# abelxiaoxing/ImageClassification

Hardware: AMD Instinct MI355X
Metric: images/sec (whole node) ResNet-50 bf16 224^2 training (higher is better)
Workload: dtype bf16; 1 GPU; resnet50 train step, synthetic 3x224x224, batch 256/GPU, AdamW, label smoothing 0.1, 1000 classes (BASELINE configs[1]); global_batch=256, parallelism=dp1

## Files before the change

imageclassification_amd/csrc/capi.hip:

```cpp
#include "../../include/icamd.h"
#include "common.h"
#include "icamd_internal.h"
#include <cstdlib>
#include <string.h>

int icamd_bn_finalize_launch(const float* part, int nrows, int C, double count, const float* gamma, const float* beta,
                             float* running_mean, float* running_var, float momentum, float eps, float* mean,
                             float* invstd, float* scale, float* shift, double* chunks, hipStream_t s);
int icamd_bn_eval_coeffs_launch(int C, const float* gamma, const float* beta, const float* rm, const float* rv, float eps,
                                float* scale, float* shift, hipStream_t s);
int icamd_bn_apply_launch(const bf16_t* y, const float* scale, const float* shift, const bf16_t* residual, bf16_t* out,
                          unsigned char* maskbits, long long numel, int C, int relu, hipStream_t s,
                          const float* res_scale = nullptr, const float* res_shift = nullptr);
int icamd_bn_bwd_rows_per_block(long long rows, int C);
int icamd_bn_bwd_launch(const bf16_t* dout, const bf16_t* act, const bf16_t* y, const float* mean, const float* invstd,
                        const float* scale, const float* shift, float* dgamma, float* dbeta, bf16_t* dy, bf16_t* gout,
                        const unsigned char* maskbits, long long rows, int C, int relu, int accumulate, float* part,
                        double* chunks, float* c1c2, hipStream_t s, const unsigned char* pool_idx = nullptr,
                        int pool_ih = 0, int pool_iw = 0);
int icamd_bn_bwd_dual_launch(const bf16_t* dout, const unsigned char* maskbits, const bf16_t* yA, const float* meanA,
                             const float* invstdA, const float* scaleA, float* dgammaA, float* dbetaA, bf16_t* dyA,
                             const bf16_t* yB, const float* meanB, const float* invstdB, const float* scaleB, float* dgammaB,
                             float* dbetaB, bf16_t* dyB, long long rows, int C, int accumulate, float* partA, double* chunksA,
                             float* cA, float* partB, double* chunksB, float* cB, hipStream_t s);
// ... 404 lines not shown
  if (!conv_desc_ok(d) || d->KH != 1 || d->KW != 1 || d->stride != 1 || d->pad != 0) return 0;
  return icamd_pw_resident_bnred_wanted((long long)d->N * d->IH * d->IW, d->Cin, d->Cout) ? 1 : 0;
}

int icamd_conv2d_dgrad_bnred(const icamd_conv_desc* d, const void* dy, const void* w_t, void* g, const void* addend,
                             const uint8_t* addend_bits, int addend_sub2, const void* bn_y, const uint8_t* bn_bits,
                             float* partials, void* stream) {
  ProfScope _prof(PC_IGEMM_DGRAD, stream);
  const ConvWork cw = conv_work(d); _prof.work(cw.out + 3 * cw.in + 2 * cw.w + cw.in / 16 + (addend_bits ? cw.in / 16 : 0), cw.flops);
  if (!conv_desc_ok(d) || dy == nullptr || w_t == nullptr || g == nullptr || addend == nullptr || bn_y == nullptr ||
      bn_bits == nullptr || partials == nullptr || (addend_sub2 && addend_bits != nullptr))
    return ICAMD_ERR_BAD_ARG;
  if (!icamd_conv2d_dgrad_bnred_supported(d)) return ICAMD_ERR_UNSUPPORTED;
  PwResidentParams p;
  memset(&p, 0, sizeof(p));
  p.A = (const bf16_t*)dy; p.B = (const bf16_t*)w_t; p.out = (bf16_t*)g; p.addend = (const bf16_t*)addend;
  p.addend_bits = addend_bits;
  p.bn_y = (const bf16_t*)bn_y; p.bn_bits = bn_bits; p.bn_part = partials;
  p.M = d->N * d->IH * d->IW; p.N = d->Cin; p.K = d->Cout;
  if (addend_sub2) { p.sub2_h = d->IH; p.sub2_w = d->IW; }
  return icamd_pw_resident_bnred_launch(p, (hipStream_t)stream);
}

size_t icamd_conv2d_wgrad_workspace_bytes(const icamd_conv_desc* d) {
  if (!conv_desc_ok(d)) return 0;
  int S = 1, rows = 0;
  const long long M = (long long)d->N * d->OH * d->OW;
  if (M >= (1ll << 30)) return 0;
  const int Ktot = d->KH * d->KW * d->Cin;
  icamd_wgrad_plan((int)M, d->Cout, Ktot, &S, &rows);
  if (icamd_wgrad_halo_wanted(d->KH, d->KW, d->stride, d->pad, d->OH, d->OW, d->Cin, d->Cout, M)) {
    int S2 = 1;
    icamd_wgrad_halo_plan((int)M, d->Cin, d->Cout, &S2, &rows);
    if (S2 > S) S = S2;
  }
  return (size_t)S * d->Cout * ((size_t)Ktot + 1) * sizeof(float);
}

static int wgrad_impl(const icamd_conv_desc* d, const void* x, const void* dy, float* dw, float* dbias, int accumulate,
                      void* workspace, size_t workspace_bytes, void* stream);

int icamd_conv2d_wgrad(const icamd_conv_desc* d, const void* x, const void* dy, float* dw, int accumulate,
                       void* workspace, size_t workspace_bytes, void* stream) {
  ProfScope _prof(PC_WGRAD, stream);
  const ConvWork cw = conv_work(d); _prof.work(cw.in + cw.out + 4 * cw.w, cw.flops);
  return wgrad_impl(d, x, dy, dw, nullptr, accumulate, workspace, workspace_bytes, stream);
// ... 861 lines not shown
```

imageclassification_amd/csrc/conv3x3_halo.hip:

```cpp
#ifndef ICAMD_C64_NT
#define ICAMD_C64_NT 0
#endif
#include "common.h"
#include "icamd_internal.h"
#include <cstdlib>

namespace {

template <int N> __device__ __forceinline__ void halo_wait_vmcnt() {
  static_assert(N >= 0 && N < 64, "vmcnt is a 6-bit field");
  asm volatile("s_waitcnt vmcnt(%0)" ::"n"(N) : "memory");
}

__device__ __forceinline__ int swzq(int blk) { return (0x78 >> (2 * blk)) & 3; }

template <int BN, int WN, int MFR, int LA, int NB, int KS, int WPS>
__global__ __launch_bounds__(256, WPS) void conv3x3_halo_kernel(const Halo3x3Params p) {
  constexpr int WM = 4 / WN;
  constexpr int BM = WM * MFR * 16;
  constexpr int NJ = BN / WN / 16;
  constexpr int A_SLOTS = 4 * LA * 8;
  constexpr int ZERO_SLOT = A_SLOTS - 1;
  constexpr int A_BYTES = A_SLOTS * 128;
  constexpr int B_STAGE = BN * KS * 2;
  constexpr int LB = BN * KS / 2048;
  static_assert(KS == 32 || KS == 64, "filter stage width");
  constexpr int RING = NB * B_STAGE;
  constexpr int EPI_BYTES = BM * BN * 2;
  constexpr int LDS_BYTES = (A_BYTES + RING > EPI_BYTES) ? A_BYTES + RING : EPI_BYTES;
  static_assert(NB >= 2 && NB <= 8 && (WN == 1 || WN == 2) && LB >= 1, "configuration");
  __shared__ __attribute__((aligned(16))) unsigned char smem[LDS_BYTES];
  unsigned char* const sA = smem;
  unsigned char* const sB = smem + A_BYTES;

  const int tid = threadIdx.x, lane = tid & 63;
  const int wave = __builtin_amdgcn_readfirstlane(tid >> 6);
  const int wm = wave % WM, wn = wave / WM;
  const int fr = lane & 15, fq = lane >> 4;

// ... 151 lines not shown
  constexpr int ROWB = BN * 2, CPR = BN / 8;
#pragma unroll
  for (int j = 0; j < NJ; ++j) {
    const int cl = wn * (BN / WN) + j * 16 + 4 * fq;
    const int cg = n0 + cl;
    const int cgc = cg < p.Cout ? cg : 0;
    f32x4 b4 = {0.f, 0.f, 0.f, 0.f};
    if (p.bias != nullptr) b4 = *(const f32x4*)(p.bias + cgc);
#pragma unroll
    for (int i = 0; i < MFR; ++i) {
      const int ml = wm * (BM / WM) + i * 16 + fr;
      f32x4 v = acc[j][i] + b4;
      if (p.relu) {
#pragma unroll
        for (int e = 0; e < 4; ++e) v[e] = v[e] < 0.f ? 0.f : v[e];
      }
      u32x2 pk;
      pk[0] = pack_bf16x2(v[0], v[1]);
      pk[1] = pack_bf16x2(v[2], v[3]);
      const int slot = cl >> 2;
      *(u32x2*)(smem + ml * ROWB + ((((slot >> 1) ^ ml) & (CPR - 1)) << 4) + ((slot & 1) << 3)) = pk;
    }
  }
  __syncthreads();
  constexpr int RPP = 256 / CPR;
  constexpr int NPASS = BM / RPP;
  const int cp = tid & (CPR - 1), rg = tid / CPR;
  const int co = n0 + cp * 8;
  const bool co_ok = co < p.Cout;
  float s1[8], s2[8];
#pragma unroll
  for (int e = 0; e < 8; ++e) { s1[e] = 0.f; s2[e] = 0.f; }
#pragma unroll
  for (int ps = 0; ps < NPASS; ++ps) {
    const int ml = ps * RPP + rg;
    const int m = m0 + ml;
    const u32x4 o = *(const u32x4*)(smem + ml * ROWB + (((cp ^ ml) & (CPR - 1)) << 4));
    if (m < p.M && co_ok) {
      *(u32x4*)(p.out + (long long)m * p.Cout + co) = o;
      if (p.stats != nullptr) {
#pragma unroll
        for (int e = 0; e < 4; ++e) {
          const float lo = bf16_lo(o[e]), hi = bf16_hi(o[e]);
          s1[2 * e] += lo; s2[2 * e] += lo * lo;
          s1[2 * e + 1] += hi; s2[2 * e + 1] += hi * hi;
        }
      }
    }
  }
  if (p.stats != nullptr) {
    __syncthreads();
    float* red = (float*)smem;
#pragma unroll
    for (int e = 0; e < 8; ++e) {
      red[(rg * 2 + 0) * BN + cp * 8 + e] = s1[e];
      red[(rg * 2 + 1) * BN + cp * 8 + e] = s2[e];
    }
    __syncthreads();
    const int ntm = (p.M + BM - 1) / BM, nrows = (p.M + 127) / 128;
    for (int idx = tid; idx < 2 * BN; idx += 256) {
      const int which = idx / BN, c = idx - which * BN;
      float s = 0.f;
#pragma unroll 4
      for (int g = 0; g < RPP; ++g) s += red[(g * 2 + which) * BN + c];
      if (n0 + c < p.Cout) {
        p.stats[((long long)tile_m * 2 + which) * p.Cout + n0 + c] = s;
        if (ntm + tile_m < nrows) p.stats[((long long)(ntm + tile_m) * 2 + which) * p.Cout + n0 + c] = 0.f;
      }
    }
  }
}

template <bool ACT>
__global__ __launch_bounds__(256, 2) void conv3x3_c64_resident_kernel(const Halo3x3Params p, const int ntiles) {
  constexpr int BM = 128, LA = 8;
  constexpr int A_BYTES = 32 * LA * 128;
  constexpr int E_BYTES = 4 * 64 * 64;
  constexpr int ZERO_SLOT = 32 * LA - 1;
  __shared__ __attribute__((aligned(16))) unsigned char smem[2 * A_BYTES + E_BYTES];

  const int tid = threadIdx.x, lane = tid & 63;
  const int wave = __builtin_amdgcn_readfirstlane(tid >> 6);
  const int wm = wave & 1, wn = wave >> 1;
  const int fr = lane & 15, fq = lane >> 4;
  const int W = p.W, H = p.H;
  const bf16_t* __restrict__ in = p.in;
  const bf16_t* zero = (const bf16_t*)icamd_zero_page;
  unsigned char* const sE = smem + 2 * A_BYTES + wave * 4096;
  const unsigned lds_base = (unsigned)(uintptr_t)LPTR(smem);

  const int a_slot = wave * 8 + (lane >> 3);
  const int a_lc = (((lane & 7) - (lane >> 3)) & 7) * 8;
  const bool a_zero_lane = a_slot == 31;
  auto stage_a = [&](int m0, unsigned char* dst) {
    const int pix0 = m0 - (W + 1) + a_slot;
    const bf16_t* src0 = in + ((long long)pix0 * 64 + a_lc);
// ... 112 lines not shown
    for (int j = 0; j < 2; ++j) {
      f32x4 b4 = {0.f, 0.f, 0.f, 0.f};
      if constexpr (ACT) {
        if (p.bias != nullptr) b4 = *(const f32x4*)(p.bias + wn * 32 + j * 16 + 4 * fq);
      }
#pragma unroll
      for (int i = 0; i < 4; ++i) {
        const int pl = i * 16 + fr;
        f32x4 v = acc[j][i];
        if constexpr (ACT) {
          v += b4;
          if (p.relu) {
#pragma unroll
            for (int e = 0; e < 4; ++e) v[e] = v[e] < 0.f ? 0.f : v[e];
          }
        }
        u32x2 pk;
        pk[0] = pack_bf16x2(v[0], v[1]);
        pk[1] = pack_bf16x2(v[2], v[3]);
        const int slot = j * 4 + fq;
        *(u32x2*)(sE + pl * 64 + ((((slot >> 1) ^ (pl >> 2)) & 3) << 4) + ((slot & 1) << 3)) = pk;
      }
    }
    {
      const int pl0 = lane >> 2;
      const int mrow = m0 + wm * 64 + pl0;
      bf16_t* orow = p.out + ((long long)mrow * 64 + wn * 32 + (lane & 3) * 8);
      const bool want_stats = p.stats != nullptr;
#pragma unroll
      for (int r = 0; r < 4; ++r) {
        const int pl = r * 16 + pl0;
        const u32x4 o = *(const u32x4*)(sE + pl * 64 + ((((lane & 3) ^ (pl >> 2)) & 3) << 4));
        if (mrow + r * 16 < p.M) {
          *(u32x4*)(orow + r * (16 * 64)) = o;
          if (want_stats) {
#pragma unroll
            for (int e = 0; e < 4; ++e) {
              const f32x2 v = {bf16_lo(o[e]), bf16_hi(o[e])};
              s1[e] += v;
              s2[e] = __builtin_elementwise_fma(v, v, s2[e]);
            }
          }
        }
      }
    }
  }

  if (p.stats != nullptr) {
    __syncthreads();
    float* red = (float*)smem;
    const int g = wm * 16 + (lane >> 2);
    const int c0 = wn * 32 + (lane & 3) * 8;
#pragma unroll
    for (int e = 0; e < 4; ++e) {
      red[(g * 2 + 0) * 64 + c0 + 2 * e] = s1[e][0];
      red[(g * 2 + 0) * 64 + c0 + 2 * e + 1] = s1[e][1];
      red[(g * 2 + 1) * 64 + c0 + 2 * e] = s2[e][0];
      red[(g * 2 + 1) * 64 + c0 + 2 * e + 1] = s2[e][1];
    }
    __syncthreads();
    if (tid < 128) {
      const int which = tid >> 6, c = tid & 63;
      float s = 0.f;
#pragma unroll 8
      for (int k = 0; k < 32; ++k) s += red[(k * 2 + which) * 64 + c];
      p.stats[((long long)blockIdx.x * 2 + which) * 64 + c] = s;
      const int nrows = (p.M + 127) / 128;
      for (int r = blockIdx.x + gridDim.x; r < nrows; r += gridDim.x) p.stats[((long long)r * 2 + which) * 64 + c] = 0.f;
    }
  }
}

int launch_resident_c64(const Halo3x3Params& p, hipStream_t stream) {
  const int ntiles = (p.M + 127) / 128;
  const int slots = 2 * icamd_num_cus();
  const int grid = ntiles < slots ? ntiles : slots;
  if (p.bias != nullptr || p.relu)
    hipLaunchKernelGGL((conv3x3_c64_resident_kernel<true>), dim3((unsigned)grid), dim3(256), 0, stream, p, ntiles);
  else
    hipLaunchKernelGGL((conv3x3_c64_resident_kernel<false>), dim3((unsigned)grid), dim3(256), 0, stream, p, ntiles);
  return icamd_launch_status();
}

template <int BN, int WN, int MFR, int LA, int NB, int KS, int WPS>
int launch_halo(const Halo3x3Params& p, hipStream_t stream) {
  constexpr int BM = (4 / WN) * MFR * 16;
  const int ntm = (p.M + BM - 1) / BM;
  hipLaunchKernelGGL((conv3x3_halo_kernel<BN, WN, MFR, LA, NB, KS, WPS>), dim3((unsigned)(ntm * p.ntiles_n)), dim3(256), 0,
                     stream, p);
  return icamd_launch_status();
}

int halo_mode() {
  static const int m = [] { const char* e = getenv("ICAMD_CONV3X3_HALO"); return e ? atoi(e) : 1; }();
  return m;
}

}

static bool resident_c64_ok(int W, int C, int Cout) {
  static const int on = [] { const char* e = getenv("ICAMD_CONV3X3_RESIDENT"); return e ? atoi(e) : 1; }();
  return on != 0 && C == 64 && Cout == 64 && W % 8 == 0 && 128 + 2 * W + 2 <= 255;
}

bool icamd_halo3x3_wanted(int N, int H, int W, int C, int Cout) {
  if (halo_mode() == 0) return false;
  if (C % 64 != 0 || Cout % 8 != 0 || W < 3 || H < 3) return false;
  if (resident_c64_ok(W, C, Cout)) return true;
  if (halo_mode() == 1 && C < 256) return false;
  if ((long long)N * H * W >= (1ll << 30)) return false;
  if (2 * W + 3 + 128 > 4 * 8 * 8) return false;
  return true;
}

int icamd_halo3x3_launch(Halo3x3Params& p, hipStream_t stream) {
  if (!icamd_halo3x3_wanted(p.N, p.H, p.W, p.C, p.Cout)) return ICAMD_ERR_UNSUPPORTED;
  p.M = p.N * p.H * p.W;
  p.divHW = make_fastdiv((unsigned)(p.H * p.W));
  p.divW = make_fastdiv((unsigned)p.W);
  if (resident_c64_ok(p.W, p.C, p.Cout)) return launch_resident_c64(p, stream);
  const int bn = p.Cout <= 64 ? 64 : 128;
  p.ntiles_n = (p.Cout + bn - 1) / bn;
  int bm = 128;
  if (halo_mode() == 3) bm = 256;
  else if (halo_mode() != 2) {
    long long best = -1;
    for (int cand : {256, 224, 128}) {
      if (cand == 224 && bn != 128) continue;
      if ((cand + 2 * p.W + 3 + 31) / 32 > (cand == 128 ? 8 : 12)) continue;
      const long long tiles = (long long)((p.M + cand - 1) / cand) * p.ntiles_n;
      const long long cost = ((tiles + 511) / 512) * cand + (cand == 128 ? 16 : 0);
      if (best < 0 || cost < best) { best = cost; bm = cand; }
    }
  }
  const bool big = bm != 128;
  const int slots = bm + 2 * p.W + 2 + 1;
  const int la = (slots + 31) / 32;
  if (la > 12) return ICAMD_ERR_UNSUPPORTED;
  if (bn == 128) {
// ... 24 lines not shown
```

imageclassification_amd/csrc/icamd_internal.h:

```cpp
#pragma once
#include "common.h"

#define ICAMD_MAX_TAPS 56

struct IgemmParams {
  const bf16_t* in;
  const bf16_t* wt;
  bf16_t* out;
  const bf16_t* addend;
  const unsigned char* addend_bits;
  int addend_sub2;
  const float* bias;
  float* stats;
  const bf16_t* bnb_y;
  const bf16_t* bnb_mask;
  const float *bnb_mean, *bnb_invstd, *bnb_scale, *bnb_shift;
  int bnb_relu;
  int relu;
  bf16_t* gelu_out;
  int gelu_inplace;
  const bf16_t* gelu_z;
  int N, IH, IW, Cin;
  int OH, OW, Cout;
  int P, Q, M;
  int ostr, ooff_h, ooff_w, istr;
  int ntaps, Ktot;
  int KW, pad;
  int tap_sign, regular_taps;
  int stem7;
  int ksteps, ntiles_n;
  FastDiv divPQ, divQ, divCin, divKW;
  short dh[ICAMD_MAX_TAPS], dw[ICAMD_MAX_TAPS], wtap[ICAMD_MAX_TAPS];
};
int icamd_igemm_launch(IgemmParams& p, hipStream_t stream);
int icamd_igemm_pick_bn(int Cout);

struct Halo3x3Params {
  const bf16_t* in;
  const bf16_t* wt;
  bf16_t* out;
  const float* bias;
  float* stats;
  int relu;
  int flip;
  int N, H, W, C, Cout;
  int M, ntiles_n;
  FastDiv divHW, divW;
};
bool icamd_halo3x3_wanted(int N, int H, int W, int C, int Cout);
int icamd_halo3x3_launch(Halo3x3Params& p, hipStream_t stream);

struct GConvParams {
  const bf16_t* in;
  const bf16_t* w;
  bf16_t* out;
  const bf16_t* dy;
  float* slab;
  const float* bias;
  float* stats;
  int relu;
  int N, IH, IW, OH, OW, C, groups, stride;
  int Cg, M, npix_in, nalloc;
  int S, tiles_per_split, ntiles;
  FastDiv divOHW, divOW;
};
bool icamd_gconv3x3_ok(int N, int IH, int IW, int OH, int OW, int C, int groups, int stride);
int icamd_gconv3x3_fwd_launch(GConvParams& p, hipStream_t stream);
int icamd_gconv3x3_dgrad_launch(GConvParams& p, hipStream_t stream);
size_t icamd_gconv3x3_wgrad_bytes(int N, int IH, int IW, int OH, int OW, int C, int groups, int stride);
int icamd_gconv3x3_wgrad_launch(GConvParams& p, hipStream_t stream);

struct GemmNtParams {
// ... 128 lines not shown
```

imageclassification_amd/hip.py:

```python
import ctypes
import os
from ctypes import POINTER, Structure, c_double, c_float, c_int, c_longlong, c_size_t, c_void_p

import torch

_HERE = os.path.dirname(os.path.abspath(__file__))
LIB_PATH = os.path.join(_HERE, "csrc", "libicamd.so")

ABI_VERSION = 6
ERRORS = {1: "ICAMD_ERR_BAD_ARG", 2: "ICAMD_ERR_UNSUPPORTED", 3: "ICAMD_ERR_WORKSPACE", 4: "ICAMD_ERR_LAUNCH"}


class IcamdError(RuntimeError):
    pass


class BnBwdFuse(Structure):
    _fields_ = [("y", c_void_p), ("mask_src", c_void_p), ("mean", c_void_p), ("invstd", c_void_p), ("scale", c_void_p),
                ("shift", c_void_p), ("partials", c_void_p), ("relu", c_int)]


class ImageDesc(Structure):
    _fields_ = [("src_offset", ctypes.c_int64), ("src_h", c_int), ("src_w", c_int), ("crop_top", c_int), ("crop_left", c_int),
                ("crop_h", c_int), ("crop_w", c_int), ("hflip", c_int), ("vflip", c_int), ("jitter_order", c_int * 3),
# ... 19 lines not shown


def conv_desc(N, IH, IW, Cin, Cout, KH, KW, stride, pad):
    OH = (IH + 2 * pad - KH) // stride + 1
    OW = (IW + 2 * pad - KW) // stride + 1
    return ConvDesc(N, IH, IW, Cin, OH, OW, Cout, KH, KW, stride, pad)


_P = c_void_p
_SIGNATURES = {
    "icamd_abi_version": (c_int, []),
    "icamd_conv2d_fwd_gelu": (c_int, [_P, _P, _P, _P, _P, _P, _P]),
    "icamd_conv2d_dgrad_gelu": (c_int, [_P, _P, _P, _P, _P, _P]),
    "icamd_conv2d_fwd_act": (c_int, [_P, _P, _P, _P, _P, _P, c_int, _P]),
    "icamd_bn_fold_filters": (c_int, [_P, _P, _P, _P, _P, c_float, c_int, c_int, _P, _P, _P]),
    "icamd_conv2d_stats_rows": (c_int, [POINTER(ConvDesc)]),
    "icamd_conv2d_fwd": (c_int, [POINTER(ConvDesc), _P, _P, _P, _P, _P, _P, _P]),
    "icamd_conv2d_dgrad": (c_int, [POINTER(ConvDesc), _P, _P, _P, _P, _P, _P]),
    "icamd_conv2d_dgrad_sub2": (c_int, [POINTER(ConvDesc), _P, _P, _P, _P, _P]),
    "icamd_conv2d_dgrad_stats_rows": (c_int, [POINTER(ConvDesc)]),
    "icamd_conv2d_dgrad_bnbwd": (c_int, [POINTER(ConvDesc), _P, _P, _P, _P, POINTER(BnBwdFuse), _P]),
    "icamd_conv2d_dgrad_bnred_supported": (c_int, [POINTER(ConvDesc)]),
    "icamd_conv2d_dgrad_bnred": (c_int, [POINTER(ConvDesc), _P, _P, _P, _P, _P, c_int, _P, _P, _P, _P]),
    "icamd_bn_bwd_from_gy_partials": (c_int, [_P, c_int, _P, _P, _P, _P, _P, _P, _P, _P, c_longlong, c_int, c_int, _P, c_size_t, _P]),
    "icamd_bn_apply_conv1x1_fused_supported": (c_int, [POINTER(ConvDesc)]),
    "icamd_bn_apply_conv1x1_fused": (c_int, [POINTER(ConvDesc), _P, _P, _P, _P, _P, _P, _P, _P, _P, _P, _P, _P]),
    "icamd_conv1x1_bn_bwd_fused_supported": (c_int, [POINTER(ConvDesc)]),
    "icamd_conv1x1_bn_bwd_fused_workspace_bytes": (c_size_t, [POINTER(ConvDesc)]),
    "icamd_conv1x1_bn_bwd_fused": (c_int, [POINTER(ConvDesc), _P, c_int, _P, _P, _P, _P, _P, _P, _P, _P, _P, _P, _P, c_int, _P, c_size_t,
                                           _P, c_size_t, _P]),
    "icamd_conv2d_wgrad_workspace_bytes": (c_size_t, [POINTER(ConvDesc)]),
    "icamd_conv2d_wgrad": (c_int, [POINTER(ConvDesc), _P, _P, _P, c_int, _P, c_size_t, _P]),
    "icamd_conv2d_wgrad_bias": (c_int, [POINTER(ConvDesc), _P, _P, _P, _P, c_int, _P, c_size_t, _P]),
    "icamd_gconv3x3_supported": (c_int, [POINTER(ConvDesc), c_int]),
    "icamd_gconv3x3_fwd": (c_int, [POINTER(ConvDesc), c_int, _P, _P, _P, _P, _P]),
    "icamd_gconv3x3_fwd_act": (c_int, [POINTER(ConvDesc), c_int, _P, _P, _P, _P, c_int, _P]),
    "icamd_gconv3x3_dgrad": (c_int, [POINTER(ConvDesc), c_int, _P, _P, _P, _P]),
    "icamd_gconv3x3_wgrad_workspace_bytes": (c_size_t, [POINTER(ConvDesc), c_int]),
    "icamd_gconv3x3_wgrad": (c_int, [POINTER(ConvDesc), c_int, _P, _P, _P, c_int, _P, c_size_t, _P]),
    "icamd_filter_transpose": (c_int, [_P, _P, _P, _P, c_int, _P]),
    "icamd_filter_transpose_tiled": (c_int, [_P, _P, _P, _P, c_int, _P]),
    "icamd_bn_workspace_bytes": (c_size_t, [c_int]),
    "icamd_bn_train_finalize": (c_int, [_P, c_int, c_int, c_double, _P, _P, _P, _P, c_float, c_float, _P, _P, _P, _P, _P, _P]),
    "icamd_bn_eval_coeffs": (c_int, [c_int, _P, _P, _P, _P, c_float, _P, _P, _P]),
    "icamd_bn_apply": (c_int, [_P, _P, _P, _P, _P, _P, c_longlong, c_int, c_int, _P]),
    "icamd_bn_apply_res_bn": (c_int, [_P, _P, _P, _P, _P, _P, _P, _P, c_longlong, c_int, c_int, _P]),
# ... 135 lines not shown
```

imageclassification_amd/nets.py:

```python
import ctypes
import math
import os
from collections import OrderedDict

import torch

from . import hip
from .checkpoint import PicklableModel

BN_EPS = 1e-5
_FUSED_BNBWD = os.environ.get("ICAMD_FUSED_BNBWD", "0") == "1"
_WGRAD_STREAM = os.environ.get("ICAMD_WGRAD_STREAM", "1") != "0"
_DUAL_BNBWD = os.environ.get("ICAMD_DUAL_BNBWD", "1") != "0"
_SUB2_SHORTCUT = os.environ.get("ICAMD_SUB2_SHORTCUT", "1") != "0"
_FUSED_POOL_BWD = os.environ.get("ICAMD_FUSED_POOL_BWD", "1") != "0"
BN_MOMENTUM = 0.1

ARCHS = {
    "resnet18": ("basic", [2, 2, 2, 2], 1, 64),
    "resnet34": ("basic", [3, 4, 6, 3], 1, 64),
    "resnet50": ("bottleneck", [3, 4, 6, 3], 1, 64),
    "resnet101": ("bottleneck", [3, 4, 23, 3], 1, 64),
    "resnet152": ("bottleneck", [3, 8, 36, 3], 1, 64),
    "wide_resnet50_2": ("bottleneck", [3, 4, 6, 3], 1, 128),
    "wide_resnet101_2": ("bottleneck", [3, 4, 23, 3], 1, 128),
    "resnext50_32x4d": ("bottleneck", [3, 4, 6, 3], 32, 4),
    "resnext101_32x4d": ("bottleneck", [3, 4, 23, 3], 32, 4),
}


def block_specs(arch):
    block, layers, cardinality, base_width = ARCHS[arch]
    expansion = 4 if block == "bottleneck" else 1
    specs = []
    inplanes = 64
    for li, (planes, nblocks) in enumerate(zip([64, 128, 256, 512], layers)):
        for bi in range(nblocks):
            stride = 2 if (bi == 0 and li > 0) else 1
# ... 417 lines not shown
        ws = self._ws.get(key)
        if ws is not None:
            return ws
        dev = self.device
        lib = self.lib
        ws = {"N": N, "H": H, "W": W}

        def act(n, h, w, c):
            return torch.empty(n, h, w, c, dtype=torch.bfloat16, device=dev)

        Ws = W + (W & 1)
        ws["Ws"] = Ws
        ws["x8"] = act(N, H, Ws + 8, 4)
        d0 = self.stem_conv.desc(N, H, Ws)
        ws["y0"] = act(N, d0.OH, d0.OW, 64)
        ws["a0"] = act(N, d0.OH, d0.OW, 64)
        PH, PW = (d0.OH - 1) // 2 + 1, (d0.OW - 1) // 2 + 1
        ws["p0"] = act(N, PH, PW, 64)
        ws["p0_idx"] = torch.empty(N, PH, PW, 64, dtype=torch.uint8, device=dev)
        max_act = max(ws["y0"].numel(), ws["x8"].numel())
        max_stats = lib.icamd_conv2d_stats_rows(ctypes.byref(d0)) * 2 * 64
        max_wg = lib.icamd_stem7x7s2_wgrad_workspace_bytes(N, H, Ws, 64)
        max_bnb = lib.icamd_bn_bwd_workspace_bytes(N * d0.OH * d0.OW, 64)
        h, w = PH, PW
        blocks_ws = []
        for blk in self.blocks:
            b = {}
            ih, iw = h, w
            ys, acts = [], []
            for ci, conv in enumerate(blk["convs"]):
                d = conv.desc(N, ih, iw)
                ys.append(act(N, d.OH, d.OW, conv.cout_p))
                acts.append(act(N, d.OH, d.OW, conv.cout_p))
                max_act = max(max_act, ys[-1].numel())
                max_stats = max(max_stats, lib.icamd_conv2d_stats_rows(ctypes.byref(d)) * 2 * conv.cout_p)
                if conv.groups > 1:
                    if not lib.icamd_gconv3x3_supported(ctypes.byref(d), conv.groups):
                        raise hip.IcamdError(f"{conv.name}: no grouped 3x3 kernel for {d.key()} with {conv.groups} groups")
                    max_wg = max(max_wg, lib.icamd_gconv3x3_wgrad_workspace_bytes(ctypes.byref(d), conv.groups))
                else:
                    max_wg = max(max_wg, lib.icamd_conv2d_wgrad_workspace_bytes(ctypes.byref(d)))
                max_bnb = max(max_bnb, lib.icamd_bn_bwd_workspace_bytes(N * d.OH * d.OW, conv.cout_p))
                ih, iw = d.OH, d.OW
            b["y"], b["a"] = ys, acts
            b["mask"] = torch.empty(acts[-1].numel() // 8, dtype=torch.uint8, device=dev)
            if "down_conv" in blk:
                dd = blk["down_conv"].desc(N, h, w)
                b["yd"] = act(N, dd.OH, dd.OW, blk["down_conv"].cout_p)
                b["ad"] = act(N, dd.OH, dd.OW, blk["down_conv"].cout_p)
                max_stats = max(max_stats, lib.icamd_conv2d_stats_rows(ctypes.byref(dd)) * 2 * blk["down_conv"].cout_p)
                max_wg = max(max_wg, lib.icamd_conv2d_wgrad_workspace_bytes(ctypes.byref(dd)))
                max_bnb = max(max_bnb, lib.icamd_bn_bwd_workspace_bytes(N * dd.OH * dd.OW, blk["down_conv"].cout_p))
            blocks_ws.append(b)
            h, w = ih, iw
        ws["blocks"] = blocks_ws
        ws["final_hw"] = (h, w)
        ws["pooled"] = torch.empty(N, self.feat_dim, dtype=torch.bfloat16, device=dev)
        ws["logits"] = torch.zeros(N, self.ncls_p, dtype=torch.bfloat16, device=dev)
        dfc = self.fc.desc(N, 1, 1)
        max_wg = max(max_wg, lib.icamd_conv2d_wgrad_workspace_bytes(ctypes.byref(dfc)))
        ws["stats"] = torch.empty(max_stats, dtype=torch.float32, device=dev)
        ws["bn_ws"] = torch.zeros(lib.icamd_bn_workspace_bytes(2048), dtype=torch.uint8, device=dev)
        ws["wgrad_ws"] = torch.empty(max_wg, dtype=torch.uint8, device=dev)
        ws["wgrad_ws_bytes"] = max_wg
        ws["bnb_part"] = torch.empty(max_stats + 4 * 2 * 2048, dtype=torch.float32, device=dev)
        ws["bna_ws_bytes"] = lib.icamd_bn_bwd_apply_workspace_bytes(2048)
        ws["bna_ws"] = torch.zeros(ws["bna_ws_bytes"], dtype=torch.uint8, device=dev)
        ws["bnb_ws"] = torch.zeros(max_bnb, dtype=torch.uint8, device=dev)
        ws["bnb_ws2"] = torch.zeros(max_bnb, dtype=torch.uint8, device=dev)
        ws["bnb_ws_bytes"] = max_bnb
        ws["max_act"] = max_act
        ws["loss_rows"] = torch.empty(N, dtype=torch.float32, device=dev)
        ws["pred"] = torch.empty(N, dtype=torch.int32, device=dev)
        ws["dlogits"] = torch.zeros(N, self.ncls_p, dtype=torch.bfloat16, device=dev)
        ws["dpooled"] = torch.empty(N, self.feat_dim, dtype=torch.bfloat16, device=dev)
        ws["scale_shift_eval"] = torch.empty(2 * 2048, dtype=torch.float32, device=dev)
        self._ws[key] = ws
        return ws

    def _grad_buffers(self, ws):
        if "gbuf" not in ws:
            n = ws["max_act"]
            ws["gbuf"] = [torch.empty(n, dtype=torch.bfloat16, device=self.device) for _ in range(8)]
        return ws["gbuf"]

    def _w(self, conv):
        return self.shadow.data_ptr() + 2 * conv.w.offset

# ... 294 lines not shown
                bnl = bns[-1]
                stl = self.stat_arena.data_ptr() + 4 * bnl.stat_offset
                cl = bnl.c
                if fuse3:
                    fused_conv_bn(convs[-1], bnl, d3, ws["bnb_part"].data_ptr(), fused_rows, b["y"][-1],
                                  b["a"][nconv - 2].data_ptr(), DA, ws["bna_ws"].data_ptr(), ws["bna_ws_bytes"])
                    fused_conv3 = True
                else:
                    hip.check(lib.icamd_bn_bwd_from_gy_partials(ws["bnb_part"].data_ptr(), fused_rows, dout, b["y"][-1].data_ptr(),
                                                                stl, stl + 4 * cl, stl + 8 * cl, self._gf(bnl.weight),
                                                                self._gf(bnl.bias), ypool[yk], b["y"][-1].numel() // cl, cl, acc,
                                                                ws["bna_ws"].data_ptr(), ws["bna_ws_bytes"], s),
                              bnl.name + " bwd (apply, sums from the data gradient)")
            else:
                bn_bwd(bns[-1], dout, None, b["y"][-1], ypool[yk], None, True, mask)
            fused_rows = 0
            for i in range(nconv - 1, 0, -1):
                x_i = b["a"][i - 1]
                if fused_conv3 and i == nconv - 1:
                    yk = next_y()
                    bn_bwd(bns[i - 1], DA, None, b["y"][i - 1], ypool[yk], None, True)
                    continue
                wgrad(convs[i], x_i.data_ptr(), ypool[yk], N, *hw_in[i], ybuf=yk)
                dgrad(convs[i], ypool[yk], DA, None, N, *hw_in[i])
                yk = next_y()
                bn_bwd(bns[i - 1], DA, None, b["y"][i - 1], ypool[yk], None, True)
            wgrad(convs[0], xin.data_ptr(), ypool[yk], N, h, w, ybuf=yk)
            if shortcut_done:
                dgrad(convs[0], ypool[yk], other, T, N, h, w)
            elif "down_conv" in blk:
                if y2 is None:
                    y2 = next_y()
                    bn_bwd(blk["down_bn"], dout, None, b["yd"], ypool[y2], None, True, mask)
                dc = blk["down_conv"]
                wgrad(dc, xin.data_ptr(), ypool[y2], N, h, w, ybuf=y2)
                if _SUB2_SHORTCUT and dc.k == 1 and dc.stride == 2 and dc.pad == 0:
                    dd = dc.desc(N, h, w)
                    key = ("sub2", N, dd.OH, dd.OW)
                    d1 = dc.descs.get(key)
                    if d1 is None:
                        d1 = dc.descs[key] = hip.conv_desc(N, dd.OH, dd.OW, dc.cin_p, dc.cout_p, 1, 1, 1, 0)
                    hip.check(lib.icamd_conv2d_dgrad(ctypes.byref(d1), ypool[y2], self._wt(dc), T, None, None, s),
                              dc.name + " dgrad (even grid)")
                    d0 = convs[0].desc(N, h, w)
                    if (prev_takes_g and self.block == "bottleneck"
                            and lib.icamd_conv2d_dgrad_bnred_supported(ctypes.byref(d0))):
# ... 170 lines not shown
```

include/icamd.h:

```cpp
#ifndef ICAMD_H
#define ICAMD_H
#include <stddef.h>
#include <stdint.h>

#ifdef __cplusplus
extern "C" {
#endif

#define ICAMD_OK 0
#define ICAMD_ERR_BAD_ARG 1
#define ICAMD_ERR_UNSUPPORTED 2
#define ICAMD_ERR_WORKSPACE 3
#define ICAMD_ERR_LAUNCH 4

int icamd_abi_version(void);

typedef struct icamd_conv_desc {
  int N, IH, IW, Cin;
  int OH, OW, Cout;
  int KH, KW, stride, pad;
} icamd_conv_desc;

int icamd_conv2d_stats_rows(const icamd_conv_desc* d);

// ... 66 lines not shown
                              const float* invstd, const float* scale, const float* shift, float* dgamma, float* dbeta,
                              void* dy, int N, int IH, int IW, int C, int accumulate, void* workspace, size_t workspace_bytes,
                              void* stream);

int icamd_bn_bwd_dual(const void* dout, const uint8_t* maskbits, const void* yA, const float* meanA, const float* invstdA,
                      const float* scaleA, float* dgammaA, float* dbetaA, void* dyA, const void* yB, const float* meanB,
                      const float* invstdB, const float* scaleB, float* dgammaB, float* dbetaB, void* dyB, long long rows, int C,
                      int accumulate, void* workspaceA, void* workspaceB, size_t workspace_bytes, void* stream);

size_t icamd_bn_bwd_apply_workspace_bytes(int C);
int icamd_bn_bwd_from_partials(const float* partials, int nrows, const void* g, const void* y, const float* mean,
                               const float* invstd, const float* scale, float* dgamma, float* dbeta, void* dy,
                               long long rows, int C, int accumulate, void* workspace, size_t workspace_bytes,
                               void* stream);

int icamd_conv2d_dgrad_bnred_supported(const icamd_conv_desc* d);
int icamd_conv2d_dgrad_bnred(const icamd_conv_desc* d, const void* dy, const void* w_t, void* g, const void* addend,
                             const uint8_t* addend_bits, int addend_sub2, const void* bn_y, const uint8_t* bn_bits,
                             float* partials, void* stream);
int icamd_bn_bwd_from_gy_partials(const float* partials, int nrows, const void* g, const void* y, const float* mean,
                                  const float* invstd, const float* scale, float* dgamma, float* dbeta, void* dy,
                                  long long rows, int C, int accumulate, void* workspace, size_t workspace_bytes,
                                  void* stream);

int icamd_bn_apply_conv1x1_fused_supported(const icamd_conv_desc* d);
int icamd_bn_apply_conv1x1_fused(const icamd_conv_desc* d, const void* y, const float* scale, const float* shift,
                                 const void* residual, const float* res_scale, const float* res_shift, void* out,
                                 uint8_t* maskbits, const void* w, void* y1, float* stats, void* stream);

int icamd_conv1x1_bn_bwd_fused_supported(const icamd_conv_desc* d);
size_t icamd_conv1x1_bn_bwd_fused_workspace_bytes(const icamd_conv_desc* d);
int icamd_conv1x1_bn_bwd_fused(const icamd_conv_desc* d, const float* partials, int nrows, const void* g, const void* y,
                               const float* mean, const float* invstd, const float* scale, float* dgamma, float* dbeta,
                               const void* x, const void* w_t, void* dx, float* dw, int accumulate, void* bn_workspace,
                               size_t bn_workspace_bytes, void* wgrad_workspace, size_t wgrad_workspace_bytes, void* stream);

int icamd_layernorm_fwd(const void* x, const float* gamma, const float* beta, void* y, float* mean, float* rstd,
                        long long rows, int C, float eps, void* stream);
size_t icamd_layernorm_bwd_workspace_bytes(long long rows, int C);
int icamd_layernorm_bwd(const void* dy, const void* x, const float* mean, const float* rstd, const float* gamma,
                        const void* addend, void* dx, float* dgamma, float* dbeta, long long rows, int C, int accumulate,
                        void* workspace, size_t workspace_bytes, void* stream);
int icamd_gelu_fwd(const void* z, void* a, long long numel, void* stream);
int icamd_gelu_bwd(const void* da, const void* z, void* dz, long long numel, void* stream);
size_t icamd_colsum_rows_workspace_bytes(long long rows, int cols);
int icamd_colsum_rows(const void* x, long long rows, int ld, int cols, float* out, int accumulate, void* workspace,
// ... 143 lines not shown
```

Measured before the change: 14520 images/sec.

## Fuse BN-ReLU mask and BN backward reductions into 3x3 halo dgrad epilogue

Adds a BN-reduce variant of the 3x3 halo and c64-resident dgrad kernels. In the epilogue each kernel recomputes the ReLU mask from the saved BN input with scale and shift, masks the data gradient, and accumulates per-channel sums of g and g*y into partials. The bottleneck's 3x3 backward then calls bn_bwd_from_gy_partials directly and skips the separate BN backward reduction pass. In exchange the epilogue gains an extra read of y plus scale and shift loads and more register pressure, and a new stats workspace is allocated.

```diff
diff --git a/imageclassification_amd/csrc/capi.hip b/imageclassification_amd/csrc/capi.hip
--- a/imageclassification_amd/csrc/capi.hip
+++ b/imageclassification_amd/csrc/capi.hip
@@ -450,6 +450,33 @@
   return icamd_pw_resident_bnred_launch(p, (hipStream_t)stream);
 }
 
+int icamd_conv3x3_dgrad_bnred_supported(const icamd_conv_desc* d) {
+  if (!conv_desc_ok(d) || d->KH != 3 || d->KW != 3 || d->stride != 1 || d->pad != 1) return 0;
+  if ((long long)d->N * d->IH * d->IW >= (1ll << 31)) return 0;
+  return icamd_halo3x3_bnred_wanted(d->N, d->IH, d->IW, d->Cout, d->Cin) ? 1 : 0;
+}
+
+int icamd_conv3x3_dgrad_bnred_stats_rows(const icamd_conv_desc* d) {
+  if (!icamd_conv3x3_dgrad_bnred_supported(d)) return 0;
+  return (int)(((long long)d->N * d->IH * d->IW + 127) / 128);
+}
+
+int icamd_conv3x3_dgrad_bnred(const icamd_conv_desc* d, const void* dy, const void* w_t, void* g, const void* bn_y,
+                              const float* bn_scale, const float* bn_shift, float* partials, void* stream) {
+  ProfScope _prof(PC_IGEMM_DGRAD, stream);
+  const ConvWork cw = conv_work(d); _prof.work(cw.out + 2 * cw.in + 2 * cw.w, cw.flops);
+  if (!conv_desc_ok(d) || dy == nullptr || w_t == nullptr || g == nullptr || bn_y == nullptr || bn_scale == nullptr ||
+      bn_shift == nullptr || partials == nullptr)
+    return ICAMD_ERR_BAD_ARG;
+  if (!icamd_conv3x3_dgrad_bnred_supported(d)) return ICAMD_ERR_UNSUPPORTED;
+  Halo3x3Params h;
+  memset(&h, 0, sizeof(h));
+  h.in = (const bf16_t*)dy; h.wt = (const bf16_t*)w_t; h.out = (bf16_t*)g; h.flip = 1;
+  h.bn_y = (const bf16_t*)bn_y; h.bn_scale = bn_scale; h.bn_shift = bn_shift; h.bn_part = partials;
+  h.N = d->N; h.H = d->IH; h.W = d->IW; h.C = d->Cout; h.Cout = d->Cin;
+  return icamd_halo3x3_launch(h, (hipStream_t)stream);
+}
+
 size_t icamd_conv2d_wgrad_workspace_bytes(const icamd_conv_desc* d) {
   if (!conv_desc_ok(d)) return 0;
   int S = 1, rows = 0;
diff --git a/imageclassification_amd/csrc/conv3x3_halo.hip b/imageclassification_amd/csrc/conv3x3_halo.hip
--- a/imageclassification_amd/csrc/conv3x3_halo.hip
+++ b/imageclassification_amd/csrc/conv3x3_halo.hip
@@ -14,7 +14,7 @@
 
 __device__ __forceinline__ int swzq(int blk) { return (0x78 >> (2 * blk)) & 3; }
 
-template <int BN, int WN, int MFR, int LA, int NB, int KS, int WPS>
+template <int BN, int WN, int MFR, int LA, int NB, int KS, int WPS, bool BNR>
 __global__ __launch_bounds__(256, WPS) void conv3x3_halo_kernel(const Halo3x3Params p) {
   constexpr int WM = 4 / WN;
   constexpr int BM = WM * MFR * 16;
@@ -212,12 +212,29 @@
       *(u32x2*)(smem + ml * ROWB + ((((slot >> 1) ^ ml) & (CPR - 1)) << 4) + ((slot & 1) << 3)) = pk;
     }
   }
-  __syncthreads();
   constexpr int RPP = 256 / CPR;
   constexpr int NPASS = BM / RPP;
   const int cp = tid & (CPR - 1), rg = tid / CPR;
   const int co = n0 + cp * 8;
   const bool co_ok = co < p.Cout;
+  u32x4 yv[BNR ? NPASS : 1];
+  float sc[8], sh[8];
+  if constexpr (BNR) {
+    const int coc = co_ok ? co : 0;
+#pragma unroll
+    for (int ps = 0; ps < NPASS; ++ps) {
+      const int m = m0 + ps * RPP + rg;
+      yv[ps] = *(const u32x4*)(p.bn_y + (long long)(m < p.M ? m : p.M - 1) * p.Cout + coc);
+    }
+#pragma unroll
+    for (int e = 0; e < 8; e += 4) {
+      const f32x4 a = *(const f32x4*)(p.bn_scale + coc + e), b = *(const f32x4*)(p.bn_shift + coc + e);
+#pragma unroll
+      for (int k = 0; k < 4; ++k) { sc[e + k] = a[k]; sh[e + k] = b[k]; }
+    }
+  }
+  float* const stats = BNR ? p.bn_part : p.stats;
+  __syncthreads();
   float s1[8], s2[8];
 #pragma unroll
   for (int e = 0; e < 8; ++e) { s1[e] = 0.f; s2[e] = 0.f; }
@@ -225,20 +242,33 @@
   for (int ps = 0; ps < NPASS; ++ps) {
     const int ml = ps * RPP + rg;
     const int m = m0 + ml;
-    const u32x4 o = *(const u32x4*)(smem + ml * ROWB + (((cp ^ ml) & (CPR - 1)) << 4));
+    u32x4 o = *(const u32x4*)(smem + ml * ROWB + (((cp ^ ml) & (CPR - 1)) << 4));
+    if constexpr (BNR) {
+#pragma unroll
+      for (int e = 0; e < 4; ++e) {
+        const unsigned int keep = (fmaf(bf16_lo(yv[ps][e]), sc[2 * e], sh[2 * e]) > 0.f ? 0x0000ffffu : 0u) |
+                                  (fmaf(bf16_hi(yv[ps][e]), sc[2 * e + 1], sh[2 * e + 1]) > 0.f ? 0xffff0000u : 0u);
+        o[e] &= keep;
+      }
+    }
     if (m < p.M && co_ok) {
       *(u32x4*)(p.out + (long long)m * p.Cout + co) = o;
-      if (p.stats != nullptr) {
+      if (stats != nullptr) {
 #pragma unroll
         for (int e = 0; e < 4; ++e) {
           const float lo = bf16_lo(o[e]), hi = bf16_hi(o[e]);
-          s1[2 * e] += lo; s2[2 * e] += lo * lo;
-          s1[2 * e + 1] += hi; s2[2 * e + 1] += hi * hi;
+          if constexpr (BNR) {
+            s1[2 * e] += lo; s2[2 * e] = fmaf(lo, bf16_lo(yv[ps][e]), s2[2 * e]);
+            s1[2 * e + 1] += hi; s2[2 * e + 1] = fmaf(hi, bf16_hi(yv[ps][e]), s2[2 * e + 1]);
+          } else {
+            s1[2 * e] += lo; s2[2 * e] += lo * lo;
+            s1[2 * e + 1] += hi; s2[2 * e + 1] += hi * hi;
+          }
         }
       }
     }
   }
-  if (p.stats != nullptr) {
+  if (stats != nullptr) {
     __syncthreads();
     float* red = (float*)smem;
 #pragma unroll
@@ -254,14 +284,14 @@
 #pragma unroll 4
       for (int g = 0; g < RPP; ++g) s += red[(g * 2 + which) * BN + c];
       if (n0 + c < p.Cout) {
-        p.stats[((long long)tile_m * 2 + which) * p.Cout + n0 + c] = s;
-        if (ntm + tile_m < nrows) p.stats[((long long)(ntm + tile_m) * 2 + which) * p.Cout + n0 + c] = 0.f;
-      }
-    }
-  }
-}
-
-template <bool ACT>
+        stats[((long long)tile_m * 2 + which) * p.Cout + n0 + c] = s;
+        if (ntm + tile_m < nrows) stats[((long long)(ntm + tile_m) * 2 + which) * p.Cout + n0 + c] = 0.f;
+      }
+    }
+  }
+}
+
+template <bool ACT, bool BNR>
 __global__ __launch_bounds__(256, 2) void conv3x3_c64_resident_kernel(const Halo3x3Params p, const int ntiles) {
   constexpr int BM = 128, LA = 8;
   constexpr int A_BYTES = 32 * LA * 128;
@@ -420,15 +450,42 @@
         *(u32x2*)(sE + pl * 64 + ((((slot >> 1) ^ (pl >> 2)) & 3) << 4) + ((slot & 1) << 3)) = pk;
       }
     }
+    u32x4 yv[BNR ? 4 : 1];
+    f32x4 sc4[2], sh4[2];
+    if constexpr (BNR) {
+      __builtin_amdgcn_sched_barrier(0);
+      const int mrow = m0 + wm * 64 + (lane >> 2);
+      const int c0 = wn * 32 + (lane & 3) * 8;
+#pragma unroll
+      for (int r = 0; r < 4; ++r) {
+        const int m = mrow + r * 16;
+        yv[r] = *(const u32x4*)(p.bn_y + ((long long)(m < p.M ? m : p.M - 1) * 64 + c0));
+      }
+#pragma unroll
+      for (int e = 0; e < 2; ++e) {
+        sc4[e] = *(const f32x4*)(p.bn_scale + c0 + 4 * e);
+        sh4[e] = *(const f32x4*)(p.bn_shift + c0 + 4 * e);
+      }
+    }
+
     {
       const int pl0 = lane >> 2;
       const int mrow = m0 + wm * 64 + pl0;
       bf16_t* orow = p.out + ((long long)mrow * 64 + wn * 32 + (lane & 3) * 8);
-      const bool want_stats = p.stats != nullptr;
+      const bool want_stats = BNR || p.stats != nullptr;
 #pragma unroll
       for (int r = 0; r < 4; ++r) {
         const int pl = r * 16 + pl0;
-        const u32x4 o = *(const u32x4*)(sE + pl * 64 + ((((lane & 3) ^ (pl >> 2)) & 3) << 4));
+        u32x4 o = *(const u32x4*)(sE + pl * 64 + ((((lane & 3) ^ (pl >> 2)) & 3) << 4));
+        if constexpr (BNR) {
+#pragma unroll
+          for (int e = 0; e < 4; ++e) {
+            const int q = e >> 1, k = (e & 1) * 2;
+            const unsigned int keep = (fmaf(bf16_lo(yv[r][e]), sc4[q][k], sh4[q][k]) > 0.f ? 0x0000ffffu : 0u) |
+                                      (fmaf(bf16_hi(yv[r][e]), sc4[q][k + 1], sh4[q][k + 1]) > 0.f ? 0xffff0000u : 0u);
+            o[e] &= keep;
+          }
+        }
         if (mrow + r * 16 < p.M) {
           *(u32x4*)(orow + r * (16 * 64)) = o;
           if (want_stats) {
@@ -436,7 +493,8 @@
             for (int e = 0; e < 4; ++e) {
               const f32x2 v = {bf16_lo(o[e]), bf16_hi(o[e])};
               s1[e] += v;
-              s2[e] = __builtin_elementwise_fma(v, v, s2[e]);
+              if constexpr (BNR) s2[e] = __builtin_elementwise_fma(v, f32x2{bf16_lo(yv[r][e]), bf16_hi(yv[r][e])}, s2[e]);
+              else s2[e] = __builtin_elementwise_fma(v, v, s2[e]);
             }
           }
         }
@@ -444,7 +502,8 @@
     }
   }
 
-  if (p.stats != nullptr) {
+  float* const stats = BNR ? p.bn_part : p.stats;
+  if (stats != nullptr) {
     __syncthreads();
     float* red = (float*)smem;
     const int g = wm * 16 + (lane >> 2);
@@ -462,9 +521,9 @@
       float s = 0.f;
 #pragma unroll 8
       for (int k = 0; k < 32; ++k) s += red[(k * 2 + which) * 64 + c];
-      p.stats[((long long)blockIdx.x * 2 + which) * 64 + c] = s;
+      stats[((long long)blockIdx.x * 2 + which) * 64 + c] = s;
       const int nrows = (p.M + 127) / 128;
-      for (int r = blockIdx.x + gridDim.x; r < nrows; r += gridDim.x) p.stats[((long long)r * 2 + which) * 64 + c] = 0.f;
+      for (int r = blockIdx.x + gridDim.x; r < nrows; r += gridDim.x) stats[((long long)r * 2 + which) * 64 + c] = 0.f;
     }
   }
 }
@@ -473,10 +532,12 @@
   const int ntiles = (p.M + 127) / 128;
   const int slots = 2 * icamd_num_cus();
   const int grid = ntiles < slots ? ntiles : slots;
-  if (p.bias != nullptr || p.relu)
-    hipLaunchKernelGGL((conv3x3_c64_resident_kernel<true>), dim3((unsigned)grid), dim3(256), 0, stream, p, ntiles);
+  if (p.bn_part != nullptr)
+    hipLaunchKernelGGL((conv3x3_c64_resident_kernel<false, true>), dim3((unsigned)grid), dim3(256), 0, stream, p, ntiles);
+  else if (p.bias != nullptr || p.relu)
+    hipLaunchKernelGGL((conv3x3_c64_resident_kernel<true, false>), dim3((unsigned)grid), dim3(256), 0, stream, p, ntiles);
   else
-    hipLaunchKernelGGL((conv3x3_c64_resident_kernel<false>), dim3((unsigned)grid), dim3(256), 0, stream, p, ntiles);
+    hipLaunchKernelGGL((conv3x3_c64_resident_kernel<false, false>), dim3((unsigned)grid), dim3(256), 0, stream, p, ntiles);
   return icamd_launch_status();
 }
 
@@ -484,8 +545,15 @@
 int launch_halo(const Halo3x3Params& p, hipStream_t stream) {
   constexpr int BM = (4 / WN) * MFR * 16;
   const int ntm = (p.M + BM - 1) / BM;
-  hipLaunchKernelGGL((conv3x3_halo_kernel<BN, WN, MFR, LA, NB, KS, WPS>), dim3((unsigned)(ntm * p.ntiles_n)), dim3(256), 0,
-                     stream, p);
+  const dim3 grid((unsigned)(ntm * p.ntiles_n));
+  if constexpr (BN == 128) {
+    if (p.bn_part != nullptr) {
+      hipLaunchKernelGGL((conv3x3_halo_kernel<BN, WN, MFR, LA, NB, KS, WPS, true>), grid, dim3(256), 0, stream, p);
+      return icamd_launch_status();
+    }
+  }
+  if (p.bn_part != nullptr) return ICAMD_ERR_UNSUPPORTED;
+  hipLaunchKernelGGL((conv3x3_halo_kernel<BN, WN, MFR, LA, NB, KS, WPS, false>), grid, dim3(256), 0, stream, p);
   return icamd_launch_status();
 }
 
@@ -511,8 +579,20 @@
   return true;
 }
 
+bool icamd_halo3x3_bnred_wanted(int N, int H, int W, int C, int Cout) {
+  if (halo_mode() == 0) return false;
+  if (C % 64 != 0 || W < 3 || H < 3) return false;
+  if (resident_c64_ok(W, C, Cout)) return true;
+  return Cout % 128 == 0 && icamd_halo3x3_wanted(N, H, W, C, Cout);
+}
+
 int icamd_halo3x3_launch(Halo3x3Params& p, hipStream_t stream) {
-  if (!icamd_halo3x3_wanted(p.N, p.H, p.W, p.C, p.Cout)) return ICAMD_ERR_UNSUPPORTED;
+  const bool bnr = p.bn_part != nullptr;
+  if (bnr && (p.bn_y == nullptr || p.bn_scale == nullptr || p.bn_shift == nullptr || p.flip != 1 || p.bias != nullptr ||
+              p.relu || p.stats != nullptr))
+    return ICAMD_ERR_BAD_ARG;
+  if (bnr ? !icamd_halo3x3_bnred_wanted(p.N, p.H, p.W, p.C, p.Cout) : !icamd_halo3x3_wanted(p.N, p.H, p.W, p.C, p.Cout))
+    return ICAMD_ERR_UNSUPPORTED;
   p.M = p.N * p.H * p.W;
   p.divHW = make_fastdiv((unsigned)(p.H * p.W));
   p.divW = make_fastdiv((unsigned)p.W);
diff --git a/imageclassification_amd/csrc/icamd_internal.h b/imageclassification_amd/csrc/icamd_internal.h
--- a/imageclassification_amd/csrc/icamd_internal.h
+++ b/imageclassification_amd/csrc/icamd_internal.h
@@ -41,6 +41,10 @@
   bf16_t* out;
   const float* bias;
   float* stats;
+  const bf16_t* bn_y;
+  const float* bn_scale;
+  const float* bn_shift;
+  float* bn_part;
   int relu;
   int flip;
   int N, H, W, C, Cout;
@@ -48,6 +52,7 @@
   FastDiv divHW, divW;
 };
 bool icamd_halo3x3_wanted(int N, int H, int W, int C, int Cout);
+bool icamd_halo3x3_bnred_wanted(int N, int H, int W, int C, int Cout);
 int icamd_halo3x3_launch(Halo3x3Params& p, hipStream_t stream);
 
 struct GConvParams {
diff --git a/imageclassification_amd/hip.py b/imageclassification_amd/hip.py
--- a/imageclassification_amd/hip.py
+++ b/imageclassification_amd/hip.py
@@ -65,6 +65,9 @@
     "icamd_conv2d_dgrad_bnbwd": (c_int, [POINTER(ConvDesc), _P, _P, _P, _P, POINTER(BnBwdFuse), _P]),
     "icamd_conv2d_dgrad_bnred_supported": (c_int, [POINTER(ConvDesc)]),
     "icamd_conv2d_dgrad_bnred": (c_int, [POINTER(ConvDesc), _P, _P, _P, _P, _P, c_int, _P, _P, _P, _P]),
+    "icamd_conv3x3_dgrad_bnred_supported": (c_int, [POINTER(ConvDesc)]),
+    "icamd_conv3x3_dgrad_bnred_stats_rows": (c_int, [POINTER(ConvDesc)]),
+    "icamd_conv3x3_dgrad_bnred": (c_int, [POINTER(ConvDesc), _P, _P, _P, _P, _P, _P, _P, _P]),
     "icamd_bn_bwd_from_gy_partials": (c_int, [_P, c_int, _P, _P, _P, _P, _P, _P, _P, _P, c_longlong, c_int, c_int, _P, c_size_t, _P]),
     "icamd_bn_apply_conv1x1_fused_supported": (c_int, [POINTER(ConvDesc)]),
     "icamd_bn_apply_conv1x1_fused": (c_int, [POINTER(ConvDesc), _P, _P, _P, _P, _P, _P, _P, _P, _P, _P, _P, _P]),
diff --git a/imageclassification_amd/nets.py b/imageclassification_amd/nets.py
--- a/imageclassification_amd/nets.py
+++ b/imageclassification_amd/nets.py
@@ -14,6 +14,7 @@
 _DUAL_BNBWD = os.environ.get("ICAMD_DUAL_BNBWD", "1") != "0"
 _SUB2_SHORTCUT = os.environ.get("ICAMD_SUB2_SHORTCUT", "1") != "0"
 _FUSED_POOL_BWD = os.environ.get("ICAMD_FUSED_POOL_BWD", "1") != "0"
+_DGRAD3X3_BNRED = os.environ.get("ICAMD_DGRAD3X3_BNRED", "1") != "0"
 BN_MOMENTUM = 0.1
 
 ARCHS = {
@@ -477,6 +478,7 @@
         max_stats = lib.icamd_conv2d_stats_rows(ctypes.byref(d0)) * 2 * 64
         max_wg = lib.icamd_stem7x7s2_wgrad_workspace_bytes(N, H, Ws, 64)
         max_bnb = lib.icamd_bn_bwd_workspace_bytes(N * d0.OH * d0.OW, 64)
+        max_dg3 = 0
         h, w = PH, PW
         blocks_ws = []
         for blk in self.blocks:
@@ -489,6 +491,8 @@
                 acts.append(act(N, d.OH, d.OW, conv.cout_p))
                 max_act = max(max_act, ys[-1].numel())
                 max_stats = max(max_stats, lib.icamd_conv2d_stats_rows(ctypes.byref(d)) * 2 * conv.cout_p)
+                if conv.k == 3 and conv.groups == 1:
+                    max_dg3 = max(max_dg3, lib.icamd_conv3x3_dgrad_bnred_stats_rows(ctypes.byref(d)) * 2 * conv.cin_p)
                 if conv.groups > 1:
                     if not lib.icamd_gconv3x3_supported(ctypes.byref(d), conv.groups):
                         raise hip.IcamdError(f"{conv.name}: no grouped 3x3 kernel for {d.key()} with {conv.groups} groups")
@@ -519,6 +523,7 @@
         ws["wgrad_ws"] = torch.empty(max_wg, dtype=torch.uint8, device=dev)
         ws["wgrad_ws_bytes"] = max_wg
         ws["bnb_part"] = torch.empty(max_stats + 4 * 2 * 2048, dtype=torch.float32, device=dev)
+        ws["dg3_part"] = torch.empty(max(max_dg3, 1), dtype=torch.float32, device=dev)
         ws["bna_ws_bytes"] = lib.icamd_bn_bwd_apply_workspace_bytes(2048)
         ws["bna_ws"] = torch.zeros(ws["bna_ws_bytes"], dtype=torch.uint8, device=dev)
         ws["bnb_ws"] = torch.zeros(max_bnb, dtype=torch.uint8, device=dev)
@@ -859,6 +864,24 @@
                     bn_bwd(bns[i - 1], DA, None, b["y"][i - 1], ypool[yk], None, True)
                     continue
                 wgrad(convs[i], x_i.data_ptr(), ypool[yk], N, *hw_in[i], ybuf=yk)
+                d_i = convs[i].desc(N, *hw_in[i])
+                if (_DGRAD3X3_BNRED and self.block == "bottleneck" and i == 1 and convs[i].groups == 1
+                        and lib.icamd_conv3x3_dgrad_bnred_supported(ctypes.byref(d_i))):
+                    bn1, y1 = bns[i - 1], b["y"][i - 1]
+                    st1 = self.stat_arena.data_ptr() + 4 * bn1.stat_offset
+                    c1 = bn1.c
+                    hip.check(lib.icamd_conv3x3_dgrad_bnred(ctypes.byref(d_i), ypool[yk], self._wt(convs[i]), DA, y1.data_ptr(),
+                                                            st1 + 8 * c1, st1 + 12 * c1, ws["dg3_part"].data_ptr(), s),
+                              convs[i].name + " dgrad + bn reduce")
+                    yk = next_y()
+                    hip.check(lib.icamd_bn_bwd_from_gy_partials(ws["dg3_part"].data_ptr(),
+                                                                lib.icamd_conv3x3_dgrad_bnred_stats_rows(ctypes.byref(d_i)), DA,
+                                                                y1.data_ptr(), st1, st1 + 4 * c1, st1 + 8 * c1,
+                                                                self._gf(bn1.weight), self._gf(bn1.bias), ypool[yk],
+                                                                y1.numel() // c1, c1, acc, ws["bna_ws"].data_ptr(),
+                                                                ws["bna_ws_bytes"], s),
+                              bn1.name + " bwd (apply, sums from the data gradient)")
+                    continue
                 dgrad(convs[i], ypool[yk], DA, None, N, *hw_in[i])
                 yk = next_y()
                 bn_bwd(bns[i - 1], DA, None, b["y"][i - 1], ypool[yk], None, True)
diff --git a/include/icamd.h b/include/icamd.h
--- a/include/icamd.h
+++ b/include/icamd.h
@@ -112,6 +112,11 @@
                                   const float* invstd, const float* scale, float* dgamma, float* dbeta, void* dy,
                                   long long rows, int C, int accumulate, void* workspace, size_t workspace_bytes,
                                   void* stream);
+
+int icamd_conv3x3_dgrad_bnred_supported(const icamd_conv_desc* d);
+int icamd_conv3x3_dgrad_bnred_stats_rows(const icamd_conv_desc* d);
+int icamd_conv3x3_dgrad_bnred(const icamd_conv_desc* d, const void* dy, const void* w_t, void* g, const void* bn_y,
+                              const float* bn_scale, const float* bn_shift, float* partials, void* stream);
 
 int icamd_bn_apply_conv1x1_fused_supported(const icamd_conv_desc* d);
 int icamd_bn_apply_conv1x1_fused(const icamd_conv_desc* d, const void* y, const float* scale, const float* shift,
```

Result: no change. 14600 images/sec (median of 6 runs) (+0.5%).
